# flair2005/image-analogies-python

Hardware: AMD Instinct MI355X
Metric: B' pixels synthesized/sec, exact NN, 1024² A/A'/B, 1/2/4/8 GPUs; % MFMA peak (higher is better)
Workload: dtype f16x3

## Files before the change

image-analogies-python_amd/_native.py:

```python
import ctypes
import math
import os
import threading

import numpy as np

_HERE = os.path.dirname(os.path.abspath(__file__))
LIB_PATH = os.environ.get('IA_LIBIA') or os.path.join(_HERE, 'libia.so')

IA_MEM_HOST, IA_MEM_DEVICE = 0, 1
IA_MATCH_F32, IA_MATCH_F16X3 = 0, 1
_ERRNAMES = {-1: 'IA_EINVAL', -2: 'IA_EHIP', -3: 'IA_ENOMEM', -4: 'IA_ENODEV', -5: 'IA_ECOMM'}


class IAError(RuntimeError):
    pass


class LevelArgs(ctypes.Structure):
    _fields_ = [('ch', ctypes.c_int), ('n_ap', ctypes.c_int), ('a_h', ctypes.c_int), ('a_w', ctypes.c_int),
                ('b_h', ctypes.c_int), ('b_w', ctypes.c_int),
                ('A', ctypes.c_void_p), ('Ac', ctypes.c_void_p), ('Ap', ctypes.c_void_p), ('Apc', ctypes.c_void_p),
                ('B', ctypes.c_void_p), ('Bc', ctypes.c_void_p), ('Bpc', ctypes.c_void_p), ('Bp', ctypes.c_void_p),
                ('weights', ctypes.c_void_p), ('kappa_factor', ctypes.c_double),
# ... 70 lines not shown
                                      ctypes.c_void_p]),
    'ia_index_destroy': (None, [ctypes.c_void_p]),
    'ia_coherence_batch': (ctypes.c_int, [ctypes.c_void_p, ctypes.c_void_p, ctypes.c_int64, ctypes.c_void_p,
                                          ctypes.c_void_p, ctypes.c_void_p, ctypes.c_int64, ctypes.c_int, ctypes.c_int,
                                          ctypes.c_int, ctypes.c_int, ctypes.c_void_p, ctypes.c_void_p,
                                          ctypes.c_void_p]),
    'ia_gaussian_pyramid': (ctypes.c_int, [ctypes.c_void_p, ctypes.c_void_p, ctypes.c_int, ctypes.c_int, ctypes.c_int,
                                           ctypes.c_int, ctypes.c_void_p, ctypes.c_void_p, ctypes.c_int]),
    'ia_color_matrix': (ctypes.c_int, [ctypes.c_void_p, ctypes.c_void_p, ctypes.c_int64, ctypes.c_void_p,
                                       ctypes.c_void_p, ctypes.c_int]),
    'ia_k3_microbench': (ctypes.c_int, [ctypes.c_void_p, ctypes.c_int64, ctypes.c_int, ctypes.c_int,
                                        ctypes.POINTER(ctypes.c_double)]),
    'ia_merge_winners': (ctypes.c_int, [ctypes.c_void_p, ctypes.c_void_p, ctypes.c_int, ctypes.c_int64,
                                        ctypes.c_void_p, ctypes.c_void_p]),
    'ia_chain_budget': (ctypes.c_int, [ctypes.c_int, ctypes.c_int, ctypes.c_int, ctypes.c_int]),
    'ia_wavefront_shape': (ctypes.c_int, [ctypes.c_int, ctypes.c_int, ctypes.POINTER(ctypes.c_int64),
                                          ctypes.POINTER(ctypes.c_int64)]),
    'ia_wavefront_step': (ctypes.c_int, [ctypes.c_int, ctypes.c_int, ctypes.c_int64, ctypes.POINTER(ctypes.c_int),
                                         ctypes.POINTER(ctypes.c_int)]),
    'ia_shard_tiles': (ctypes.c_int, [ctypes.c_int64, ctypes.c_int, ctypes.c_int, ctypes.POINTER(ctypes.c_int64),
                                      ctypes.POINTER(ctypes.c_int64)]),
    'ia_shard_tiles_pruned': (ctypes.c_int, [ctypes.c_int64, ctypes.c_int, ctypes.c_int,
                                             ctypes.POINTER(ctypes.c_int64), ctypes.POINTER(ctypes.c_int64)]),
    'ia_shard_morton_tile': (ctypes.c_int64, [ctypes.c_int64, ctypes.c_int64, ctypes.c_int]),
}

_lib = None
_lock = threading.Lock()


# ... 287 lines not shown
TILE_MUL = 2654435761


def shard_rows(n_rows, world, rank):
    t0, t1 = shard_tiles(n_rows, world, rank)
    nt = (n_rows + 31) // 32
    perm = np.arange(t0, t1, dtype=np.int64) * (TILE_MUL % nt) % nt
    rows = (np.arange(32)[:, None] * nt + perm[None, :]).ravel()
    return np.sort(rows[rows < n_rows])


def chain_budget(n_cu, vgprs, api_blocks_per_cu, wg_threads=64):
    return lib().ia_chain_budget(n_cu, vgprs, api_blocks_per_cu, wg_threads)


def wavefront_shape(h, w):
    s, m = ctypes.c_int64(), ctypes.c_int64()
    check(lib().ia_wavefront_shape(h, w, ctypes.byref(s), ctypes.byref(m)), 'ia_wavefront_shape')
    return s.value, m.value
```

image-analogies-python_amd/csrc/ia_capi.cpp:

```cpp
#include <hip/hip_runtime.h>
#include <rccl/rccl.h>

#include <algorithm>
#include <atomic>
#include <chrono>
#include <mutex>
#include <thread>
#include <cmath>
#include <cstdio>
#include <cstdlib>
#include <cstring>
#include <string>
#include <vector>

#include "../../include/ia.h"
#include "ia_internal.h"
#include "ia_launch.h"

#if IA_PROBE & 16
void ia_k3p_probe_dump();
#endif

namespace {

// ... 89 lines not shown
  int prune = 1;
  int row_source = 0;
  int shard_emulate = 1;
  int shard_unpruned = 0;
  int prune_group = 1;
  int matcher = IA_MATCH_F16X3;
  int k3p_variant = 24;
  int k3_variant = 1;
  int k3p_blocks = 1;
  int fuse_gather = 1;
  int fuse_unpruned = 0;
  HandSlot *hand = nullptr;
  int hand_rows = 0;
  int prefetch_next = 1;
  int early_gather = 1;
  int nn_bound = 1;
  int fuse_sort = 0;
  int chain_budget = 0;
  int scan_wgs = IA_NWG_H;
  unsigned long long *kslot = nullptr;
  int kslot_n = 0;
  unsigned hseq = 0;
  int time_dist = 0;
  int stamps = 0;
  int rec_wt = 1;
  DevBuf stamp_k3, stamp_mg, stamp_dur;
  std::vector<hipEvent_t> evs, evg, evm;
  hipEvent_t lv0 = nullptr, lv1 = nullptr, lv2 = nullptr;
  hipEvent_t kb[4] = {nullptr, nullptr, nullptr, nullptr};
  int rank = 0, world = 1;
// ... 273 lines not shown
  if (!std::strcmp(name, "fuse_gather")) {
    if (value != 0 && value != 1) return fail(IA_EINVAL, "ia_set_option: fuse_gather must be 0 or 1");
    c->fuse_gather = value;
    return IA_OK;
  }
  if (!std::strcmp(name, "nn_bound")) {
    if (value != 0 && value != 1) return fail(IA_EINVAL, "ia_set_option: nn_bound must be 0 or 1");
    c->nn_bound = value;
    return IA_OK;
  }
  if (!std::strcmp(name, "early_gather")) {
    if (value != 0 && value != 1) return fail(IA_EINVAL, "ia_set_option: early_gather must be 0 or 1");
    c->early_gather = value;
    return IA_OK;
  }
  if (!std::strcmp(name, "prefetch_next")) {
    if (value != 0 && value != 1) return fail(IA_EINVAL, "ia_set_option: prefetch_next must be 0 or 1");
    c->prefetch_next = value;
    return IA_OK;
  }
  if (!std::strcmp(name, "fuse_sort")) {
    if (value < 0 || value > 2) return fail(IA_EINVAL, "ia_set_option: fuse_sort must be 0, 1 or 2");
    c->fuse_sort = value;
    return IA_OK;
  }
  if (!std::strcmp(name, "fuse_unpruned")) {
    if (value != 0 && value != 1) return fail(IA_EINVAL, "ia_set_option: fuse_unpruned must be 0 or 1");
    c->fuse_unpruned = value;
    return IA_OK;
  }
// ... 156 lines not shown
  return IA_OK;
}

int ia_pipeline_generation(ia_ctx *c) { return c ? c->p_gen.load() : -1; }

int ia_chain_budget(int n_cu, int vgprs, int api_blocks_per_cu, int wg_threads) {
  if (n_cu <= 0 || vgprs <= 0 || api_blocks_per_cu <= 0 || wg_threads <= 0) return 0;
  const int alloc = (vgprs + 7) / 8 * 8;
  const int per_simd = alloc > 512 ? 0 : std::min(8, 512 / alloc);
  const int wpb = (wg_threads + IA_WAVE - 1) / IA_WAVE;
  int per_cu = std::min(4 * per_simd, api_blocks_per_cu * wpb);
  if (per_simd > 3) per_cu = std::min(per_cu, (api_blocks_per_cu - 1) * wpb);
  if (per_cu <= 0) return 0;
  const int slots = per_cu * n_cu;
  return 2 * slots - (2 * slots) / 16;
}
int ia_wavefront_shape(int h, int w, int64_t *steps, int64_t *max_queries) {
  if (h < 1 || w < 1) return fail(IA_EINVAL, "ia_wavefront_shape: empty level");
  if (steps) *steps = (int64_t)w + 3 * (int64_t)(h - 1);
  if (max_queries) *max_queries = std::min<int64_t>(h, (w + 2) / 3);
  return IA_OK;
}

int ia_wavefront_step(int h, int w, int64_t t, int *r0, int *M) {
  if (h < 1 || w < 1 || t < 0 || t >= (int64_t)w + 3 * (int64_t)(h - 1)) return fail(IA_EINVAL, "ia_wavefront_step: bad step");
  const int64_t r_lo = std::max<int64_t>(0, (t - w + 1 + 2) / 3);
  const int64_t r_hi = std::min<int64_t>(h - 1, t / 3);
  *r0 = (int)r_lo;
  *M = (int)(r_hi - r_lo + 1);
  return IA_OK;
// ... 558 lines not shown

struct LevelRun {
  ia_ctx *c;
  const LevelPlan &P;
  const LevelGeo &g;
  const LevelInputs &in;
  StampSlots &stamps;
  PipelineLink &link;
  ScanTally tally;
  double ufac;
  MergeArgs ma;
  std::vector<MergeArgs> mas;
  std::vector<int64_t> shard_rows;
  bool chain = false;
  ChainReservation &chain_res;
  bool fsort = false;
  int64_t gathered = -1;
  bool gsort = false;
  int64_t n_gm = 0;
  double gq_bytes = 0., gather_bytes_timed = 0.;

  LevelRun(ia_ctx *ctx, const LevelPlan &plan, const LevelInputs &inputs, StampSlots &s, PipelineLink &l, ChainReservation &r,
           double uf)
      : c(ctx), P(plan), g(plan.g), in(inputs), stamps(s), link(l), tally{ctx, plan.stride}, ufac(uf), chain_res(r) {}

  void init_merge_args() {
    const bool prune = P.prune, use_h = P.use_h;
    ma.db64 = c->db64.as<double>();
    ma.rec = c->rec.as<float4>();
    ma.recT = c->recT.as<float>();
// ... 32 lines not shown
      }
      for (int t = x.t0; t < x.t1 && !prune; t++) {
        const int64_t tr = ia_tile_perm(t, g.n_tiles);
        shard_rows[i] += std::min<int64_t>(IA_TILE, (g.NA - tr + g.n_tiles - 1) / g.n_tiles);
      }
    }
    gq_bytes = 55.0 * g.ch * 8 + (prune ? 12.0 * ia_db64_stride(g.ch) * 8 : 0.) + g.D * 8.0 +
               (use_h ? 16.0 * g.KS * 4 : P.DP * 4.0) + 8.0 + (prune ? 48.0 : 0.);
  }

  int init_chain() {
    static_assert(IA_NWG_H <= 4 * IA_WAVE, "k_merge_gather reads 4 records per lane");
    const int J = P.J;
    chain = c->fuse_gather && P.use_h && g.ch == 1 && g.bw >= 3 && (P.prune || c->fuse_unpruned) &&
            ((!P.multi && !P.xo && mas[0].nwg <= 4 * IA_WAVE) || (P.xo && P.prune));
    if (chain && !chain_res.take((int)(P.Mpad_max + J) + (P.xo ? 1 : 0), c->chain_budget)) chain = false;
    if (chain) {
      int rc;
      if ((rc = grow_uncached(c, (void **)&c->hand, &c->hand_rows, g.bh * J, sizeof(HandSlot))) ||
          (rc = grow_uncached(c, (void **)&c->kslot, &c->kslot_n, P.Mpad_max, 8)) || (rc = c->xerr.ensure(4)))
        return rc;
      HIP_TRY(hipMemsetAsync(c->xerr.p, 0, 4, c->st));
    }
    fsort = chain && P.prune && !P.xo && (c->fuse_sort == 1 || (c->fuse_sort == 2 && P.Mtmax >= IA_FUSE_SORT_MINQ)) &&
            g_chain_waves.load() <= c->chain_budget / 2;
    const int64_t n_timed = P.stride ? (P.T + P.stride - 1) / P.stride : 0;
    for (auto *v : {&c->evs, &c->evg, &c->evm})
      if ((int64_t)v->size() < 2 * n_timed) {
        size_t old = v->size();
        v->resize(2 * n_timed);
        for (size_t i = old; i < v->size(); i++) hipEventCreate(&(*v)[i]);
      }
    return IA_OK;
  }

  QBufs qhalf(int64_t t) const {
    const size_t h = chain && (t & 1) ? 1 : 0;
    return QBufs{c->q64.as<double>() + h * P.Mpad_max * g.D, c->qn2.as<double>() + h * P.Mpad_max,
                 P.prune ? c->qinfo.as<float4>() + h * 3 * P.Mpad_max : nullptr};
  }
// ... 10 lines not shown
    nx.sn = sn;
    const QBufs q = qhalf(sn.t);
    nx.q64 = q.q64 + q0n * g.D;
    nx.qn2 = q.qn2 + q0n;
    nx.qinfo = q.qinfo ? q.qinfo + 3 * q0n : nullptr;
    nx.qf = (char *)c->qf.p + q0n * P.db_row_bytes;
    nx.mu = c->mu.as<double>();
    nx.basis = c->pr_basis.as<double>();
    nx.ufac = ufac;
    nx.hand = c->hand + (size_t)jl * g.bh;
    nx.seq = ++c->hseq;
    nx.err = c->xerr.as<unsigned>();
    nx.timeout_ticks = IA_WAIT_TICKS;
    nx.prefetch = c->prefetch_next;
    nx.early = c->early_gather;
    return nx;
  }

  int step(int64_t t) {
    StepDesc sd;
    sd.t = (int)t;
    sd.J = P.J;
    ia_wavefront_step(g.bh, g.bw, t, &sd.r0, &sd.M);
    if (sd.M <= 0) return IA_OK;
    const int Mt = P.J * sd.M;
    sd.Mpad = (int)tile_pad(Mt);
    const bool timed_gm = P.stride && t % P.stride == 0;
    if (timed_gm) {
      hipEventRecord(c->evg[2 * n_gm], c->st);
      gather_bytes_timed += gq_bytes * Mt;
// ... 857 lines not shown
```

image-analogies-python_amd/csrc/ia_gather.h:

```cpp
#pragma once
#include "ia_dev.h"

template <int KS>
__device__ __forceinline__ void put_qh(_Float16 *qf, int m, int f, double v) {
  const int qt = m / IA_TILE, j = m % IA_TILE, s = f >> 4, h = (f >> 3) & 1, e = f & 7;
  _Float16 hi, lo;
  split_h(v, hi, lo);
  const int64_t base = (((int64_t)qt * 2 * KS + 2 * s) * IA_WAVE + h * IA_TILE + j) * 8 + e;
  qf[base] = hi;
  qf[base + IA_WAVE * 8] = lo;
}

struct QHand {
  int r0 = -1, c0 = -1, r1 = -1, c1 = -1;
  double v0 = 0., v1 = 0.;
  int s0r = 0, s0c = 0, i0 = 0, s1r = 0, s1c = 0, i1 = 0;
  int n0 = -1, n1 = -1;
};
template <bool FUSE>
__device__ __forceinline__ double feat_q1(const Imgs &B, int f, int r, int c, const QHand &h) {
  if constexpr (FUSE) {
    if (f >= 43) {
      const int k = f - 43, y = ia_reflect(r + k / 5 - 2, B.h), x = ia_reflect(c + k % 5 - 2, B.w);
      if (y == h.r0 && x == h.c0) return h.v0;
// ... 401 lines not shown
    nx.qn2[mn] = ss;
    nx.qinfo[3 * mn] = make_float4(round_down_f(p[0] - IA_PRUNE_MABS), round_down_f(p[1] - IA_PRUNE_MABS),
                                   round_down_f(p[2] - IA_PRUNE_MABS), round_down_f(p[3] - IA_PRUNE_MABS));
    nx.qinfo[3 * mn + 1] = make_float4(round_up_f(p[0] + IA_PRUNE_MABS), round_up_f(p[1] + IA_PRUNE_MABS),
                                       round_up_f(p[2] + IA_PRUNE_MABS), round_up_f(p[3] + IA_PRUNE_MABS));
    nx.qinfo[3 * mn + 2] = make_float4(up, __uint_as_float(key), z, w);
  }
  IA_GST2(5);
#if IA_PROBE & 8
  if (gprobe && lane == 0)
    printf("ESTAMP bw=%d t=%d M=%d pre=%llu part=%llu handoff=%llu late=%llu rec=%llu\n", g.bw, sn.t, sn.M, gst[1] - gst[0],
           gst[2] - gst[1], gst[3] - gst[2], gst[4] - gst[3], gst[5] - gst[4]);
#endif
#undef IA_GST2
}
```

image-analogies-python_amd/csrc/ia_internal.h:

```cpp
#pragma once
#include <hip/hip_runtime.h>
#include <stdint.h>

#define IA_WAVE 64
#define IA_TILE 32
#define IA_WG 256
#define IA_MAX_D 168
#define IA_WG_TARGET 512
#define IA_PAD_NORM 1.0e30f
#define IA_WGH 512
#define IA_NWG_H 256
#define IA_NORM_SCALE 256.0
#define IA_F16_MAXABS 64.0

template <int KS>
struct TileFmt {
  static constexpr bool CMP = KS == 4;
  static constexpr int STRIDE = CMP ? (2 * KS - 2) * IA_WAVE + 2 * IA_TILE : 2 * KS * IA_WAVE;
  __host__ __device__ static constexpr int off(int p, int L) {
    return (CMP && p >= 2 * KS - 2) ? (2 * KS - 2) * IA_WAVE + (p - (2 * KS - 2)) * IA_TILE + (L & 31) : p * IA_WAVE + L;
  }
};
#define IA_MATCH_F32 0
#define IA_MATCH_F16X3 1
// ... 212 lines not shown
  const double *mu, *basis;
  double *q64, *qn2;
  void *qf;
  float4 *qinfo;
  double ufac;
  HandSlot *hand;
  unsigned seq;
  unsigned *err;
  long long timeout_ticks;
  XOPub xp;
  const unsigned *wait_seq;
  int wait_n;
  unsigned long long *kslot;
  int prefetch;
  int early;
  int *sorder;
  float4 *sinfo;
  void *sfrag;
};

__host__ __device__ inline int ia_reflect(int i, int n) {
  int j = i < 0 ? -i - 1 : i;
  j = j >= n ? 2 * n - 1 - j : j;
  if ((unsigned)j < (unsigned)n) return j;
  const int m = 2 * n;
  i %= m;
  if (i < 0) i += m;
  return i >= n ? m - 1 - i : i;
}

// ... 12 lines not shown
```

image-analogies-python_amd/csrc/ia_kernels.hip:

```cpp
#include "ia_certify.h"
#include "ia_gather.h"
#include "ia_launch.h"

#if IA_PROBE & 8
#define IA_STAMP(k) do { __builtin_amdgcn_sched_barrier(0); stamp[k] = __builtin_amdgcn_s_memtime(); \
                         __builtin_amdgcn_sched_barrier(0); } while (0)
#else
#define IA_STAMP(k) do { } while (0)
#endif

struct MergeOut {
  double v;
  int pr, pc, img;
  int nn;
};

struct NoPre {
  __device__ __forceinline__ void operator()() const {}
};
template <int CH, int RPL, class Pre = NoPre>
__device__ __forceinline__ void merge_fused(const LevelGeo &g, const StepDesc &sd, const Imgs &A, const MergeArgs &a,
                                            int m, const JobPtrs &jp, const QPix &px,
                                            double *qs, double *ws, int *cand_row, float *cand_v,
                                            MergeOut *out = nullptr, Pre pre = Pre{}) {
#if IA_PROBE & 8
  unsigned long long stamp[8] = {0, 0, 0, 0, 0, 0, 0, 0};
#endif
  IA_STAMP(0);
  constexpr int NCOH = 15, NRR = IA_WAVE - NCOH;
  const int lane = threadIdx.x & 63;
  const int r = px.r, c = px.c, qi = px.qi;
  int32_t *__restrict__ s = jp.s, *__restrict__ im = jp.im;
  double *__restrict__ Bp = jp.Bp;
// ... 88 lines not shown
    const int pos = placed + lane_prefix(bal);
    if (cmask != 0 && pos < NRR) {
      float v;
      cand_row[pos] = lowest_cand<RPL>(cmask, i1, i2, v1, v2, v);
      cand_v[pos] = v;
      cmask &= cmask - 1;
    }
    placed += __popcll(bal);
    bal = __ballot(cmask != 0);
  }
  const int n_cand = min(placed, NRR);
  __builtin_amdgcn_wave_barrier();
  int my_row = lane < NCOH ? crow : (lane - NCOH < n_cand ? cand_row[lane - NCOH] : -1);
  const float my_v = lane >= NCOH && my_row >= 0 ? cand_v[lane - NCOH] : FLT_MAX;
  IA_STAMP(2);
  pre();

  double unw = DBL_MAX, wsq = 0.;
  double av[CH];
#pragma unroll
  for (int k = 0; k < CH; k++) av[k] = 0.;
  if (my_row >= 0) {
    const unsigned img = (unsigned)my_row / hw;
    const double *src = A.p3 + img * A.img_stride_f + (int64_t)((unsigned)my_row - img * hw) * CH;
#pragma unroll
    for (int k = 0; k < CH; k++) av[k] = src[k];
    row_dists<CH>(a.db64, my_row, qs, ws, unw, wsq);
  }
  const bool viol = lane >= NCOH && my_row >= 0 && fabs(unw - qn2 - (double)my_v) > eps + 1e-13 * (unw + qn2);
  const bool any_viol = __ballot(viol) != 0;
#if IA_PROBE & 8
// ... 169 lines not shown
      o[1] = app_pc;
      o[2] = app_img;
      o[3] = has_coh ? r - 2 + kk / 5 : 0;
      o[4] = has_coh ? c - 2 + kk % 5 : 0;
      o[5] = has_coh ? 1 : 0;
      jp.dbg_dist[2 * qi] = dbg_app;
      jp.dbg_dist[2 * qi + 1] = dbg_coh;
    }
  }
  if (out) {
    out->v = val[0];
    out->pr = pr;
    out->pc = pc;
    out->img = img;
    out->nn = bi >= 0 && bi < a.NA ? bi : -1;
  }
#if IA_PROBE & 8
  if (lane == 0 && m == sd.M / 2 && (sd.t % 256) == 128) {
    __builtin_amdgcn_s_waitcnt(0);
    const unsigned long long t7 = __builtin_amdgcn_s_memtime();
    printf("STAMP bw=%d t=%d M=%d slot=%d nfb=%d d1=%llu d2=%llu d3=%llu d4=%llu d5=%llu d6=%llu d7=%llu\n", g.bw, sd.t,
           sd.M, placed, (int)nfb, stamp[1] - stamp[0], stamp[2] - stamp[1], stamp[3] - stamp[2], stamp[4] - stamp[3],
           stamp[5] - stamp[4], stamp[6] - stamp[5], t7 - stamp[6]);
  }
#endif
}

template <int CH, bool FUSED, class JS, int RPL = IA_WG_TARGET / IA_WAVE>
__global__ void __launch_bounds__(IA_PQ_WG) k_merge_level(LevelGeo g, StepDesc sd, Imgs A, MergeArgs ma, Winner *__restrict__ win,
                                                        JS jobs) {
// ... 8 lines not shown
    const int wv = threadIdx.x >> 6;
    const unsigned long long t0 = ma.stamp ? ia_clock() : 0ull;
    merge_fused<CH, RPL>(g, sd, A, ma, m, jp, px, qsh[wv], wsh[wv], crsh[wv], cvsh[wv]);
    if (ma.stamp && (threadIdx.x & 63) == 0) ia_stamp_wg(ma.stamp, t0);
  } else {
    const double *q = ma.q64 + (int64_t)m * Geo<CH>::D;
    unsigned stat = 0;
    const Winner wn = certified_winner<RPL>(ma, m, [&](int64_t row) { return exact_dist_level<CH>(ma.db64, row, q); }, &stat);
    if ((threadIdx.x & 63) == 0) {
      win[m] = wn;
      if (jp.pstat) jp.pstat[px.qi] = stat;
    }
  }
}

template <int RPL, bool PR, bool XO, class JS>
__device__ __forceinline__ void merge_gather_body(const LevelGeo &g, const StepDesc &sd, const Imgs &A, const MergeArgs &ma,
                                                  const JS &jobs, Imgs B, const NextStep &nx) {
  constexpr int KS = 4;
  const int w = __builtin_amdgcn_readfirstlane(blockIdx.x * IA_PQ_WPB + (threadIdx.x >> 6));
  const int lane = threadIdx.x & 63, wv = threadIdx.x >> 6;
  const int J = JS::single ? 1 : sd.J, JM = J * sd.M;
  __shared__ double qsh[IA_PQ_WPB][Geo<1>::DS], wsh[IA_PQ_WPB][Geo<1>::DS];
  __shared__ int crsh[IA_PQ_WPB][IA_WAVE];
  __shared__ float cvsh[IA_PQ_WPB][IA_WAVE];
  __shared__ __attribute__((aligned(16))) _Float16 xh[IA_PQ_WPB][2][16 * KS];
  if (XO && w >= JM + J + (nx.sn.Mpad - J * nx.sn.M)) {
    if (__hip_atomic_load(nx.err, __ATOMIC_RELAXED, __HIP_MEMORY_SCOPE_AGENT)) return;
    const long long t0 = (long long)__builtin_amdgcn_s_memrealtime();
    for (int i = lane; i < nx.wait_n; i += IA_WAVE)
      while (__hip_atomic_load(nx.wait_seq + i, __ATOMIC_RELAXED, __HIP_MEMORY_SCOPE_SYSTEM) != nx.xp.seq) {
        if ((long long)__builtin_amdgcn_s_memrealtime() - t0 > nx.timeout_ticks) {
          atomicOr(nx.err, 4u);
          break;
        }
        __builtin_amdgcn_s_sleep(2);
      }
    return;
  }
  QHand h;
  int mn = -1;
  int job = 0;
  QPre pf;
  const bool early = PR && !XO && !nx.kslot && nx.prefetch && nx.early;
  QConst qk;
  if (early) qk = qconst_load(nx, lane);
#if IA_PROBE & 8
  unsigned long long gs[5] = {__builtin_amdgcn_s_memtime(), 0, 0, 0, 0}, gst[5] = {0, 0, 0, 0, 0};
  const bool gprobe = w == sd.M / 2 && (sd.t % 256) == 128 && JM == sd.M;
#endif
  if (w < JM) {
    const QPix px = ia_qpix(sd, g.bw, w);
    job = px.job;
    const JobPtrs jp = jobs.get(job);
    MergeOut o;
    if (px.c + 1 < g.bw) mn = job * nx.sn.M + (px.r - nx.sn.r0);
    const Imgs Bj = JS::single ? B : job_imgs(B, jp);
    auto pre = [&]() {
      if (PR && nx.prefetch && mn >= 0) pf = qpre_load(g, nx.sn, Bj, jp, mn, lane);
    };
    merge_fused<1, RPL>(g, sd, A, ma, w, jp, px, qsh[wv], wsh[wv], crsh[wv], cvsh[wv], &o, pre);
    if (px.r + 1 < g.bh && px.c >= 2) {
      HandSlot *hs = nx.hand + (int64_t)job * g.bh + px.r;
      if (lane == 0) {
        hs->v = o.v;
        hs->sr = o.pr;
        hs->sc = o.pc;
        hs->im = o.img;
        hs->nn = o.nn;
      }
      ia_stores_done();
      if (lane == 0) __hip_atomic_store(&hs->seq, nx.seq, __ATOMIC_RELAXED, __HIP_MEMORY_SCOPE_SYSTEM);
    }
// ... 73 lines not shown
                             );
    if (XO && nx.xp.W) xo_publish<KS>(nx.xp, mn, lane, xh[wv][0], xh[wv][1], o0, o1, o2);
    if (!XO && nx.kslot) sorted_publish<KS>(nx, mn, lane, xh[wv][0], xh[wv][1], o0, o1, o2);
  } else {
    gather_h_query_fused<KS>(g, nx.sn, B, mn, lane, nx.mu, nx.q64, nx.qn2, qf, h);
  }
#if IA_PROBE & 8
  __builtin_amdgcn_s_waitcnt(0);
  gs[3] = __builtin_amdgcn_s_memtime();
  if (gprobe && lane == 0)
    printf("GSTAMP bw=%d t=%d M=%d merge=%llu handoff_wait=%llu gather=%llu [feat+frag=%llu sums=%llu urow=%llu rec=%llu]\n",
           g.bw, sd.t, sd.M, gs[1] - gs[0], gs[2] - gs[1], gs[3] - gs[2], gst[1] - gst[0], gst[2] - gst[1], gst[3] - gst[2],
           gst[4] - gst[3]);
#endif
}
template <int RPL, bool PR, bool XO, class JS>
__global__ void __launch_bounds__(IA_PQ_WG) k_merge_gather(LevelGeo g, StepDesc sd, Imgs A, MergeArgs ma, JS jobs,
                                                         Imgs B, NextStep nx) {
  const unsigned long long t0 = ma.stamp ? ia_clock() : 0ull;
  merge_gather_body<RPL, PR, XO, JS>(g, sd, A, ma, jobs, B, nx);
  if (ma.stamp && (threadIdx.x & 63) == 0) ia_stamp_wg(ma.stamp, t0);
}

void ia_launch_merge(const LevelGeo &g, const StepDesc &sd, const Imgs &A, const MergeArgs &ma, Winner *win,
                     const JobSet &jobs, bool fused, hipStream_t st) {
  const dim3 grid(cdiv(sd.J * sd.M, IA_PQ_WPB));
  const bool r4 = fused && ma.nwg <= 4 * IA_WAVE;
  with_ch(g.ch, [&](auto c) {
    with_jobs(jobs, [&](auto js) {
      constexpr int CH = decltype(c)::CH;
      using JS = decltype(js);
      if (r4) hipLaunchKernelGGL((k_merge_level<CH, true, JS, 4>), grid, dim3(IA_PQ_WG), 0, st, g, sd, A, ma, win, js);
      else if (fused) hipLaunchKernelGGL((k_merge_level<CH, true, JS>), grid, dim3(IA_PQ_WG), 0, st, g, sd, A, ma, win, js);
      else hipLaunchKernelGGL((k_merge_level<CH, false, JS>), grid, dim3(IA_PQ_WG), 0, st, g, sd, A, ma, win, js);
    });
  });
}

struct MergeGatherInst {
  bool single, pruned, xo;
  const void *fn;
};
static const MergeGatherInst k_merge_gather_insts[] = {
    {true, true, true, (const void *)k_merge_gather<4, true, true, JobArg1>},
    {true, true, false, (const void *)k_merge_gather<4, true, false, JobArg1>},
    {true, false, false, (const void *)k_merge_gather<4, false, false, JobArg1>},
    {false, true, false, (const void *)k_merge_gather<4, true, false, JobArgN>},
    {false, false, false, (const void *)k_merge_gather<4, false, false, JobArgN>},
};

void ia_launch_merge_gather(const LevelGeo &g, const StepDesc &sd, const Imgs &A, const MergeArgs &ma, const JobSet &jobs,
                            const Imgs &B, const NextStep &nx, bool pruned, hipStream_t st) {
  const int nw = sd.J * sd.M + sd.J + (nx.sn.Mpad - sd.J * nx.sn.M) + (nx.wait_n > 0 ? 1 : 0);
  const dim3 grid(cdiv(nw, IA_PQ_WPB));
  const bool single = jobs.J == 1;
  const bool xo = single && pruned && (nx.xp.W > 0 || nx.wait_n > 0);
  for (const MergeGatherInst &k : k_merge_gather_insts) {
    if (k.single != single || k.pruned != pruned || k.xo != xo) continue;
    JobArg1 j1{jobs.j0};
    JobArgN jn{jobs.rest};
    Imgs Bj = single ? job0_imgs(B, jobs) : B;
    void *args[] = {(void *)&g,  (void *)&sd, (void *)&A, (void *)&ma, single ? (void *)&j1 : (void *)&jn,
                    (void *)&Bj, (void *)&nx};
    (void)hipLaunchKernel(k.fn, grid, dim3(IA_PQ_WG), args, 0, st);
    return;
  }
}
void ia_merge_gather_occupancy(int *vgprs, int *blocks_per_cu, int *wg_threads) {
  int vmax = 0, bmin = 1 << 30;
  for (const MergeGatherInst &k : k_merge_gather_insts) {
    hipFuncAttributes fa;
    int nb = 0;
    if (hipFuncGetAttributes(&fa, k.fn) != hipSuccess ||
        hipOccupancyMaxActiveBlocksPerMultiprocessor(&nb, k.fn, IA_PQ_WG, 0) != hipSuccess) {
      bmin = 0;
      continue;
    }
    vmax = std::max(vmax, (int)fa.numRegs);
    bmin = std::min(bmin, nb);
  }
  *vgprs = vmax;
  *blocks_per_cu = bmin;
  *wg_threads = IA_PQ_WG;
}
```

include/ia.h:

```cpp
#ifndef IA_H_
#define IA_H_

#include <stdint.h>

#ifdef __cplusplus
extern "C" {
#endif

#define IA_OK 0
#define IA_EINVAL -1
#define IA_EHIP -2
#define IA_ENOMEM -3
#define IA_ENODEV -4
#define IA_ECOMM -5

#define IA_MEM_HOST 0
#define IA_MEM_DEVICE 1

typedef struct ia_ctx ia_ctx;
typedef struct ia_index ia_index;

typedef struct {
  int64_t pixels;
  int64_t steps;
// ... 90 lines not shown
void ia_index_destroy(ia_index *index);
int ia_coherence_batch(ia_index *index, const double *q, int64_t nq, const int32_t *px,
                       const int32_t *s, const int32_t *im, int64_t n_s, int a_h, int a_w,
                       int bp_w, int pad, int32_t *p_out, int32_t *img_out, int32_t *rstar_out);

int ia_gaussian_pyramid(ia_ctx *ctx, const double *img, int h, int w, int ch, int n_reduce,
                        const double *weights7, double *out, int mem);
int ia_color_matrix(ia_ctx *ctx, const double *in, int64_t npx, const double *M9, double *out,
                    int mem);

int ia_k3_microbench(ia_ctx *ctx, int64_t n_rows, int M, int reps, double *us_per_launch);

int ia_merge_winners(const double *dist, const int64_t *row, int world, int64_t nq,
                     double *dist_out, int64_t *row_out);
int ia_chain_budget(int n_cu, int vgprs, int api_blocks_per_cu, int wg_threads);
int ia_wavefront_shape(int h, int w, int64_t *steps, int64_t *max_queries);
int ia_wavefront_step(int h, int w, int64_t t, int *r0, int *M);
int ia_shard_tiles(int64_t n_rows, int world, int rank, int64_t *tile0, int64_t *tile1);
int ia_shard_tiles_pruned(int64_t n_rows, int world, int rank, int64_t *tile0, int64_t *tile1);
int64_t ia_shard_morton_tile(int64_t storage_tile, int64_t n_tiles, int world);

#ifdef __cplusplus
}
#endif
#endif
```

Measured before the change: 5.771 million.

## Add two-wave merge/gather kernel form overlapping next-query gather with merge

```diff
diff --git a/image-analogies-python_amd/_native.py b/image-analogies-python_amd/_native.py
--- a/image-analogies-python_amd/_native.py
+++ b/image-analogies-python_amd/_native.py
@@ -108,6 +108,7 @@
     'ia_merge_winners': (ctypes.c_int, [ctypes.c_void_p, ctypes.c_void_p, ctypes.c_int, ctypes.c_int64,
                                         ctypes.c_void_p, ctypes.c_void_p]),
     'ia_chain_budget': (ctypes.c_int, [ctypes.c_int, ctypes.c_int, ctypes.c_int, ctypes.c_int]),
+    'ia_chain_choice': (ctypes.c_int, [ctypes.c_int, ctypes.c_int, ctypes.c_int, ctypes.c_int]),
     'ia_wavefront_shape': (ctypes.c_int, [ctypes.c_int, ctypes.c_int, ctypes.POINTER(ctypes.c_int64),
                                           ctypes.POINTER(ctypes.c_int64)]),
     'ia_wavefront_step': (ctypes.c_int, [ctypes.c_int, ctypes.c_int, ctypes.c_int64, ctypes.POINTER(ctypes.c_int),
@@ -425,6 +426,10 @@
     return lib().ia_chain_budget(n_cu, vgprs, api_blocks_per_cu, wg_threads)
 
 
+def chain_choice(level_waves, in_flight, budget, two_wave=1):
+    return lib().ia_chain_choice(level_waves, in_flight, budget, two_wave)
+
+
 def wavefront_shape(h, w):
     s, m = ctypes.c_int64(), ctypes.c_int64()
     check(lib().ia_wavefront_shape(h, w, ctypes.byref(s), ctypes.byref(m)), 'ia_wavefront_shape')
diff --git a/image-analogies-python_amd/csrc/ia_capi.cpp b/image-analogies-python_amd/csrc/ia_capi.cpp
--- a/image-analogies-python_amd/csrc/ia_capi.cpp
+++ b/image-analogies-python_amd/csrc/ia_capi.cpp
@@ -127,6 +127,7 @@
   int hand_rows = 0;
   int prefetch_next = 1;
   int early_gather = 1;
+  int gather_wave = 1;
   int nn_bound = 1;
   int fuse_sort = 0;
   int chain_budget = 0;
@@ -430,6 +431,11 @@
     c->early_gather = value;
     return IA_OK;
   }
+  if (!std::strcmp(name, "gather_wave")) {
+    if (value != 0 && value != 1) return fail(IA_EINVAL, "ia_set_option: gather_wave must be 0 or 1");
+    c->gather_wave = value;
+    return IA_OK;
+  }
   if (!std::strcmp(name, "prefetch_next")) {
     if (value != 0 && value != 1) return fail(IA_EINVAL, "ia_set_option: prefetch_next must be 0 or 1");
     c->prefetch_next = value;
@@ -616,6 +622,12 @@
   if (per_cu <= 0) return 0;
   const int slots = per_cu * n_cu;
   return 2 * slots - (2 * slots) / 16;
+}
+int ia_chain_choice(int level_waves, int in_flight, int budget, int two_wave) {
+  if (level_waves <= 0 || in_flight < 0 || budget <= 0) return 0;
+  const int64_t left = (int64_t)budget - in_flight;
+  if (two_wave && 2 * (int64_t)level_waves <= left) return 2;
+  return level_waves <= left ? 1 : 0;
 }
 int ia_wavefront_shape(int h, int w, int64_t *steps, int64_t *max_queries) {
   if (h < 1 || w < 1) return fail(IA_EINVAL, "ia_wavefront_shape: empty level");
@@ -1204,6 +1216,7 @@
   std::vector<int64_t> shard_rows;
   bool chain = false;
   ChainReservation &chain_res;
+  bool gwave = false;
   bool fsort = false;
   int64_t gathered = -1;
   bool gsort = false;
@@ -1266,7 +1279,15 @@
     const int J = P.J;
     chain = c->fuse_gather && P.use_h && g.ch == 1 && g.bw >= 3 && (P.prune || c->fuse_unpruned) &&
             ((!P.multi && !P.xo && mas[0].nwg <= 4 * IA_WAVE) || (P.xo && P.prune));
-    if (chain && !chain_res.take((int)(P.Mpad_max + J) + (P.xo ? 1 : 0), c->chain_budget)) chain = false;
+    const bool want_sort = P.prune && !P.xo && (c->fuse_sort == 1 || (c->fuse_sort == 2 && P.Mtmax >= IA_FUSE_SORT_MINQ));
+    const bool two = c->gather_wave && c->early_gather && c->prefetch_next && P.prune && !P.multi && !P.xo && J == 1 && !want_sort;
+    if (chain) {
+      const int lw = (int)(P.Mpad_max + J) + (P.xo ? 1 : 0);
+      int form = ia_chain_choice(lw, g_chain_waves.load(), c->chain_budget, two);
+      while (form && !chain_res.take(form * lw, c->chain_budget)) form--;
+      chain = form > 0;
+      gwave = form == 2;
+    }
     if (chain) {
       int rc;
       if ((rc = grow_uncached(c, (void **)&c->hand, &c->hand_rows, g.bh * J, sizeof(HandSlot))) ||
@@ -1274,8 +1295,7 @@
         return rc;
       HIP_TRY(hipMemsetAsync(c->xerr.p, 0, 4, c->st));
     }
-    fsort = chain && P.prune && !P.xo && (c->fuse_sort == 1 || (c->fuse_sort == 2 && P.Mtmax >= IA_FUSE_SORT_MINQ)) &&
-            g_chain_waves.load() <= c->chain_budget / 2;
+    fsort = chain && want_sort && g_chain_waves.load() <= c->chain_budget / 2;
     const int64_t n_timed = P.stride ? (P.T + P.stride - 1) / P.stride : 0;
     for (auto *v : {&c->evs, &c->evg, &c->evm})
       if ((int64_t)v->size() < 2 * n_timed) {
@@ -1316,6 +1336,7 @@
     nx.timeout_ticks = IA_WAIT_TICKS;
     nx.prefetch = c->prefetch_next;
     nx.early = c->early_gather;
+    nx.gwave = gwave;
     return nx;
   }
 
diff --git a/image-analogies-python_amd/csrc/ia_gather.h b/image-analogies-python_amd/csrc/ia_gather.h
--- a/image-analogies-python_amd/csrc/ia_gather.h
+++ b/image-analogies-python_amd/csrc/ia_gather.h
@@ -439,3 +439,219 @@
 #endif
 #undef IA_GST2
 }
+
+struct GatherWave {
+  QConst qk;
+  bool late0 = false, late1 = false;
+  bool own = false;
+  unsigned long long lm0 = 0, lm1 = 0;
+  int crow = -1;
+  double qc = 0., ss = 0., p[IA_NPC] = {0., 0., 0., 0.};
+  double part = 0., al[12] = {0., 0., 0., 0., 0., 0., 0., 0., 0., 0., 0., 0.};
+  int row2 = -1;
+  double part2 = 0., al2[12] = {0., 0., 0., 0., 0., 0., 0., 0., 0., 0., 0., 0.};
+#if IA_PROBE & 8
+  unsigned long long t0 = 0, t1 = 0, t2 = 0;
+#endif
+};
+__device__ __forceinline__ void gather_wave_row(const double *__restrict__ db64, int crow, const double *qsh,
+                                                unsigned long long lm, double &part, double *al) {
+  constexpr int D = 55, DS = Geo<1>::DS;
+  double2 rowv[DS / 2];
+  const double2 *src = reinterpret_cast<const double2 *>(db64 + (int64_t)(crow >= 0 ? crow : 0) * DS);
+#pragma unroll
+  for (int i = 0; i < DS / 2; i++) rowv[i] = src[i];
+  const double *rv = reinterpret_cast<const double *>(rowv);
+  part = pw_sum<D>([&](int f) {
+    const double d = rv[f] - qsh[f];
+    return ((lm >> f) & 1ull) ? 0. : d * d;
+  });
+#pragma unroll
+  for (int k = 0; k < 12; k++) al[k] = rv[43 + k];
+}
+template <int KS>
+__device__ __forceinline__ GatherWave gather_wave_pre(const LevelGeo &g, const NextStep &nx, const Imgs &B, const JobPtrs &jp,
+                                                      int mn, int lane, const double *__restrict__ db64, double *qsh) {
+  constexpr int D = 55, KD = 16 * KS;
+  static_assert(KD <= IA_WAVE, "one feature per lane");
+  GatherWave w;
+#if IA_PROBE & 8
+  w.t0 = __builtin_amdgcn_s_memtime();
+#endif
+  w.qk = qconst_load(nx, lane);
+  const QPre pf = qpre_load(g, nx.sn, B, jp, mn, lane);
+  const QPix pn = ia_qpix(nx.sn, g.bw, mn);
+  const int r = pn.r, c = pn.c, qi = pn.qi;
+  const bool above = r >= 1 && c + 2 < g.bw;
+  const int ar = r - 1, ac = c + 2, orr = r, oc = c - 1;
+  if (lane >= 43 && lane < D) {
+    const int k = lane - 43, y = ia_reflect(r + k / 5 - 2, B.h), x = ia_reflect(c + k % 5 - 2, B.w);
+    w.late0 = y == orr && x == oc;
+    w.late1 = above && y == ar && x == ac;
+  }
+  w.lm0 = __ballot(w.late0);
+  w.lm1 = __ballot(w.late1);
+  const bool late = w.late0 || w.late1;
+  const bool nnl = jp.nn && lane >= 15 && lane < 30;
+  if (qi > 0 && (lane < 15 || nnl)) {
+    const int k = lane < 15 ? lane : lane - 15;
+    const int nr = r - 2 + k / 5, nc = c - 2 + k % 5;
+    if (nr >= 0 && nc >= 0 && nc < g.bw && nr * g.bw + nc < qi && !(above && nr == ar && nc == ac)) {
+      if (nr == orr && nc == oc) w.own = true;
+      else w.crow = ucand_row(g, r, c, nr, nc, nnl, pf.sr, pf.sc, pf.si, pf.nn);
+    }
+  }
+  if (lane < D) qsh[lane] = late ? 0. : pf.v;
+  if (lane < KD) {
+    if (lane < D) {
+      if (!late) {
+        nx.q64[(int64_t)mn * D + lane] = pf.v;
+        w.qc = pf.v - w.qk.mu;
+        w.ss = w.qc * w.qc;
+        put_qh<KS>((_Float16 *)nx.qf, mn, lane, -2.0 * w.qc);
+#pragma unroll
+        for (int i = 0; i < IA_NPC; i++) w.p[i] = w.qk.bas[i] * w.qc;
+      }
+    } else {
+      put_qh<KS>((_Float16 *)nx.qf, mn, lane, lane == D ? IA_NORM_SCALE : 0.);
+    }
+  }
+  w.ss = wave_sum_d_x(w.ss);
+#pragma unroll
+  for (int i = 0; i < IA_NPC; i++) w.p[i] = wave_sum_d_x(w.p[i]);
+  __builtin_amdgcn_wave_barrier();
+#if IA_PROBE & 8
+  __builtin_amdgcn_s_waitcnt(0);
+  w.t1 = __builtin_amdgcn_s_memtime();
+#endif
+  gather_wave_row(db64, w.crow, qsh, w.lm0 | w.lm1, w.part, w.al);
+#if IA_PROBE & 8
+  __builtin_amdgcn_s_waitcnt(0);
+  w.t2 = __builtin_amdgcn_s_memtime();
+#endif
+  return w;
+}
+__device__ __forceinline__ void gather_wave_next(const LevelGeo &g, const NextStep &nx, const int *prow, int *prow_on,
+                                                 int lane, const double *__restrict__ db64, const double *qsh,
+                                                 GatherWave &w) {
+  const long long t0 = (long long)__builtin_amdgcn_s_memrealtime();
+  bool ok = true;
+  while (__hip_atomic_load(prow_on, __ATOMIC_ACQUIRE, __HIP_MEMORY_SCOPE_WORKGROUP) != 1) {
+    if ((long long)__builtin_amdgcn_s_memrealtime() - t0 > nx.timeout_ticks) {
+      atomicOr(nx.err, 16u);
+      ok = false;
+      break;
+    }
+    __builtin_amdgcn_s_sleep(1);
+  }
+  if (ok) {
+    const int mr = prow[lane];
+    if (mr >= 0 && mr < g.NA && (unsigned)mr % (unsigned)g.aw + 1 < (unsigned)g.aw) w.row2 = mr + 1;
+  }
+  gather_wave_row(db64, w.row2, qsh, w.lm0 | w.lm1, w.part2, w.al2);
+#if IA_PROBE & 8
+  __builtin_amdgcn_s_waitcnt(0);
+  w.t2 = __builtin_amdgcn_s_memtime();
+#endif
+}
+__device__ __forceinline__ void gather_wave_late(GatherWave &w, unsigned long long lm, double v) {
+#pragma unroll
+  for (int k = 0; k < 12; k++) {
+    if ((lm >> (43 + k)) & 1ull) {
+      const double qcl = readlane_d(w.qc, 43 + k);
+      w.ss += qcl * qcl;
+#pragma unroll
+      for (int i = 0; i < IA_NPC; i++) w.p[i] += readlane_d(w.qk.bas[i], 43 + k) * qcl;
+      const double d = w.al[k] - v;
+      w.part += d * d;
+    }
+  }
+}
+template <int KS>
+__device__ __forceinline__ void gather_wave_post(const LevelGeo &g, const NextStep &nx, const JobPtrs &jp, int job, int mn,
+                                                 int lane, const double *__restrict__ db64, const double *qsh, const QHand &h,
+                                                 int src_lane, int app_lane, GatherWave &w) {
+  constexpr int D = 55;
+#if IA_PROBE & 8
+  unsigned long long gst[5] = {__builtin_amdgcn_s_memtime(), 0, 0, 0, 0};
+  const bool gprobe = mn == nx.sn.M / 2 && (nx.sn.t % 256) == 129;
+#define IA_GST3(k) do { if (gprobe) { __builtin_amdgcn_s_waitcnt(0); __builtin_amdgcn_sched_barrier(0); \
+                        gst[k] = __builtin_amdgcn_s_memtime(); __builtin_amdgcn_sched_barrier(0); } } while (0)
+#else
+#define IA_GST3(k) do { } while (0)
+#endif
+  const QPix pn = ia_qpix(nx.sn, g.bw, mn);
+  const int r = pn.r, c = pn.c;
+  const bool above = r >= 1 && c + 2 < g.bw;
+  const int from = lane < 15 ? src_lane : app_lane;
+  const int fl = from >= 0 ? from : lane;
+  const int row2 = __shfl(w.row2, fl, 64);
+  const double part2 = __shfl(w.part2, fl, 64);
+  double al2[12];
+#pragma unroll
+  for (int k = 0; k < 12; k++) al2[k] = __shfl(w.al2[k], fl, 64);
+  if (w.own) {
+    w.crow = ucand_row(g, r, c, h.r0, h.c0, lane >= 15, h.s0r, h.s0c, h.i0, h.n0);
+    if (from >= 0 && row2 == w.crow) {
+      w.part = part2;
+#pragma unroll
+      for (int k = 0; k < 12; k++) w.al[k] = al2[k];
+    } else {
+      gather_wave_row(db64, w.crow, qsh, w.lm0 | w.lm1, w.part, w.al);
+    }
+  }
+  if (w.late0) {
+    nx.q64[(int64_t)mn * D + lane] = h.v0;
+    w.qc = h.v0 - w.qk.mu;
+    put_qh<KS>((_Float16 *)nx.qf, mn, lane, -2.0 * w.qc);
+  }
+  gather_wave_late(w, w.lm0, h.v0);
+  IA_GST3(1);
+  if (above) {
+    const HandSlot *hs = nx.hand + (int64_t)job * g.bh + (r - 1);
+    const long long t0 = (long long)__builtin_amdgcn_s_memrealtime();
+    while (__hip_atomic_load(&hs->seq, __ATOMIC_RELAXED, __HIP_MEMORY_SCOPE_SYSTEM) != nx.seq) {
+      if ((long long)__builtin_amdgcn_s_memrealtime() - t0 > nx.timeout_ticks) {
+        atomicOr(nx.err, 16u);
+        break;
+      }
+      __builtin_amdgcn_s_sleep(1);
+    }
+    const double v1 = hs->v;
+    IA_GST3(2);
+    if (w.late1) {
+      nx.q64[(int64_t)mn * D + lane] = v1;
+      w.qc = v1 - w.qk.mu;
+      put_qh<KS>((_Float16 *)nx.qf, mn, lane, -2.0 * w.qc);
+    }
+    gather_wave_late(w, w.lm1, v1);
+  } else {
+    IA_GST3(2);
+  }
+  double u = w.crow >= 0 ? w.part : DBL_MAX;
+  u = wave_min_d_x(u);
+  IA_GST3(3);
+  const double ss = w.ss, qn = sqrt(ss);
+  const double(&p)[IA_NPC] = w.p;
+  const bool fin = u < DBL_MAX;
+  const unsigned key = fin ? prune_key(p, w.qk.sc) : IA_PRUNE_KEY_INF;
+  const float up = fin ? round_up_f(u * nx.ufac) : INFINITY;
+  const float z = fin ? round_up_f((double)up - ss + 0x1p-22 * (ss + (double)up) + 0x1p-24 * (16.0 * qn + 300.0)) : INFINITY;
+  const float wd = round_up_f(0x1p-8 * qn * (1.0 + 0x1p-40));
+  if (lane == 0) {
+    nx.qn2[mn] = ss;
+    nx.qinfo[3 * mn] = make_float4(round_down_f(p[0] - IA_PRUNE_MABS), round_down_f(p[1] - IA_PRUNE_MABS),
+                                   round_down_f(p[2] - IA_PRUNE_MABS), round_down_f(p[3] - IA_PRUNE_MABS));
+    nx.qinfo[3 * mn + 1] = make_float4(round_up_f(p[0] + IA_PRUNE_MABS), round_up_f(p[1] + IA_PRUNE_MABS),
+                                       round_up_f(p[2] + IA_PRUNE_MABS), round_up_f(p[3] + IA_PRUNE_MABS));
+    nx.qinfo[3 * mn + 2] = make_float4(up, __uint_as_float(key), z, wd);
+  }
+  IA_GST3(4);
+#if IA_PROBE & 8
+  if (gprobe && lane == 0)
+    printf("WSTAMP bw=%d t=%d M=%d pre=%llu part=%llu wait_merge=%llu own=%llu handoff=%llu late=%llu rec=%llu\n", g.bw,
+           nx.sn.t, nx.sn.M, w.t1 - w.t0, w.t2 - w.t1, gst[0] - w.t2, gst[1] - gst[0], gst[2] - gst[1], gst[3] - gst[2],
+           gst[4] - gst[3]);
+#endif
+#undef IA_GST3
+}
diff --git a/image-analogies-python_amd/csrc/ia_internal.h b/image-analogies-python_amd/csrc/ia_internal.h
--- a/image-analogies-python_amd/csrc/ia_internal.h
+++ b/image-analogies-python_amd/csrc/ia_internal.h
@@ -250,6 +250,7 @@
   unsigned long long *kslot;
   int prefetch;
   int early;
+  int gwave;
   int *sorder;
   float4 *sinfo;
   void *sfrag;
diff --git a/image-analogies-python_amd/csrc/ia_kernels.hip b/image-analogies-python_amd/csrc/ia_kernels.hip
--- a/image-analogies-python_amd/csrc/ia_kernels.hip
+++ b/image-analogies-python_amd/csrc/ia_kernels.hip
@@ -13,10 +13,11 @@
   double v;
   int pr, pc, img;
   int nn;
+  int src_lane, app_lane;
 };
 
 struct NoPre {
-  __device__ __forceinline__ void operator()() const {}
+  __device__ __forceinline__ void operator()(int) const {}
 };
 template <int CH, int RPL, class Pre = NoPre>
 __device__ __forceinline__ void merge_fused(const LevelGeo &g, const StepDesc &sd, const Imgs &A, const MergeArgs &a,
@@ -135,7 +136,7 @@
   int my_row = lane < NCOH ? crow : (lane - NCOH < n_cand ? cand_row[lane - NCOH] : -1);
   const float my_v = lane >= NCOH && my_row >= 0 ? cand_v[lane - NCOH] : FLT_MAX;
   IA_STAMP(2);
-  pre();
+  pre(my_row);
 
   double unw = DBL_MAX, wsq = 0.;
   double av[CH];
@@ -335,6 +336,8 @@
     out->pc = pc;
     out->img = img;
     out->nn = bi >= 0 && bi < a.NA ? bi : -1;
+    out->src_lane = src_lane;
+    out->app_lane = recompute_app ? -1 : app_lane;
   }
 #if IA_PROBE & 8
   if (lane == 0 && m == sd.M / 2 && (sd.t % 256) == 128) {
@@ -373,17 +376,83 @@
   }
 }
 
-template <int RPL, bool PR, bool XO, class JS>
+template <int RPL>
+__device__ __forceinline__ void merge_gather_pair(const LevelGeo &g, const StepDesc &sd, const Imgs &A, const MergeArgs &ma,
+                                                  const JobPtrs &jp, const Imgs &B, const NextStep &nx, int w, int role,
+                                                  int lane, double *qsh, double *wsh, int *crsh, float *cvsh) {
+  constexpr int KS = 4;
+  __shared__ double gq[Geo<1>::DS];
+  __shared__ MergeOut mo;
+  const QPix px = ia_qpix(sd, g.bw, w);
+  const int mn = px.c + 1 < g.bw ? px.r - nx.sn.r0 : -1;
+  const bool on = mn >= 0 && mn < nx.sn.M;
+  __shared__ int prow[IA_WAVE];
+  __shared__ int prow_on;
+  if (role == 0 && lane == 0) __hip_atomic_store(&prow_on, 0, __ATOMIC_RELAXED, __HIP_MEMORY_SCOPE_WORKGROUP);
+  __syncthreads();
+  GatherWave gw;
+  MergeOut o;
+  if (role == 0) {
+    auto post = [&](int my_row) {
+      prow[lane] = my_row;
+      __builtin_amdgcn_wave_barrier();
+      if (lane == 0) __hip_atomic_store(&prow_on, 1, __ATOMIC_RELEASE, __HIP_MEMORY_SCOPE_WORKGROUP);
+    };
+    merge_fused<1, RPL>(g, sd, A, ma, w, jp, px, qsh, wsh, crsh, cvsh, &o, post);
+    if (lane == 0) mo = o;
+  } else if (on) {
+    gw = gather_wave_pre<KS>(g, nx, B, jp, mn, lane, ma.db64, gq);
+    gather_wave_next(g, nx, prow, &prow_on, lane, ma.db64, gq, gw);
+  }
+  __syncthreads();
+  if (role == 0) {
+    if (px.r + 1 < g.bh && px.c >= 2) {
+      HandSlot *hs = nx.hand + px.r;
+      if (lane == 0) {
+        hs->v = o.v;
+        hs->sr = o.pr;
+        hs->sc = o.pc;
+        hs->im = o.img;
+        hs->nn = o.nn;
+      }
+      ia_stores_done();
+      if (lane == 0) __hip_atomic_store(&hs->seq, nx.seq, __ATOMIC_RELAXED, __HIP_MEMORY_SCOPE_SYSTEM);
+    }
+    return;
+  }
+  if (!on) return;
+  QHand h;
+  h.r0 = px.r;
+  h.c0 = px.c;
+  h.v0 = mo.v;
+  h.s0r = __builtin_amdgcn_readfirstlane(mo.pr);
+  h.s0c = __builtin_amdgcn_readfirstlane(mo.pc);
+  h.i0 = __builtin_amdgcn_readfirstlane(mo.img);
+  h.n0 = __builtin_amdgcn_readfirstlane(mo.nn);
+  gather_wave_post<KS>(g, nx, jp, 0, mn, lane, ma.db64, gq, h, __builtin_amdgcn_readfirstlane(mo.src_lane),
+                       __builtin_amdgcn_readfirstlane(mo.app_lane), gw);
+}
+
+template <int RPL, bool PR, bool XO, class JS, bool GW = false>
 __device__ __forceinline__ void merge_gather_body(const LevelGeo &g, const StepDesc &sd, const Imgs &A, const MergeArgs &ma,
                                                   const JS &jobs, Imgs B, const NextStep &nx) {
   constexpr int KS = 4;
-  const int w = __builtin_amdgcn_readfirstlane(blockIdx.x * IA_PQ_WPB + (threadIdx.x >> 6));
-  const int lane = threadIdx.x & 63, wv = threadIdx.x >> 6;
+  static_assert(!GW || (PR && !XO && JS::single && IA_PQ_WPB == 1), "two-wave form: the one-job pruned early path");
+  const int w = __builtin_amdgcn_readfirstlane(GW ? blockIdx.x : blockIdx.x * IA_PQ_WPB + (threadIdx.x >> 6));
+  const int lane = threadIdx.x & 63, wv = GW ? 0 : threadIdx.x >> 6;
   const int J = JS::single ? 1 : sd.J, JM = J * sd.M;
   __shared__ double qsh[IA_PQ_WPB][Geo<1>::DS], wsh[IA_PQ_WPB][Geo<1>::DS];
   __shared__ int crsh[IA_PQ_WPB][IA_WAVE];
   __shared__ float cvsh[IA_PQ_WPB][IA_WAVE];
   __shared__ __attribute__((aligned(16))) _Float16 xh[IA_PQ_WPB][2][16 * KS];
+  if constexpr (GW) {
+    const int role = __builtin_amdgcn_readfirstlane(threadIdx.x >> 6);
+    if (w < JM) {
+      merge_gather_pair<RPL>(g, sd, A, ma, jobs.get(0), B, nx, w, role, lane, qsh[0], wsh[0], crsh[0], cvsh[0]);
+      return;
+    }
+    if (role) return;
+  }
   if (XO && w >= JM + J + (nx.sn.Mpad - J * nx.sn.M)) {
     if (__hip_atomic_load(nx.err, __ATOMIC_RELAXED, __HIP_MEMORY_SCOPE_AGENT)) return;
     const long long t0 = (long long)__builtin_amdgcn_s_memrealtime();
@@ -408,14 +477,14 @@
   unsigned long long gs[5] = {__builtin_amdgcn_s_memtime(), 0, 0, 0, 0}, gst[5] = {0, 0, 0, 0, 0};
   const bool gprobe = w == sd.M / 2 && (sd.t % 256) == 128 && JM == sd.M;
 #endif
-  if (w < JM) {
+  if (!GW && w < JM) {
     const QPix px = ia_qpix(sd, g.bw, w);
     job = px.job;
     const JobPtrs jp = jobs.get(job);
     MergeOut o;
     if (px.c + 1 < g.bw) mn = job * nx.sn.M + (px.r - nx.sn.r0);
     const Imgs Bj = JS::single ? B : job_imgs(B, jp);
-    auto pre = [&]() {
+    auto pre = [&](int) {
       if (PR && nx.prefetch && mn >= 0) pf = qpre_load(g, nx.sn, Bj, jp, mn, lane);
     };
     merge_fused<1, RPL>(g, sd, A, ma, w, jp, px, qsh[wv], wsh[wv], crsh[wv], cvsh[wv], &o, pre);
@@ -519,11 +588,11 @@
            gst[4] - gst[3]);
 #endif
 }
-template <int RPL, bool PR, bool XO, class JS>
-__global__ void __launch_bounds__(IA_PQ_WG) k_merge_gather(LevelGeo g, StepDesc sd, Imgs A, MergeArgs ma, JS jobs,
-                                                         Imgs B, NextStep nx) {
+template <int RPL, bool PR, bool XO, class JS, bool GW = false>
+__global__ void __launch_bounds__(GW ? 2 * IA_WAVE : IA_PQ_WG)
+k_merge_gather(LevelGeo g, StepDesc sd, Imgs A, MergeArgs ma, JS jobs, Imgs B, NextStep nx) {
   const unsigned long long t0 = ma.stamp ? ia_clock() : 0ull;
-  merge_gather_body<RPL, PR, XO, JS>(g, sd, A, ma, jobs, B, nx);
+  merge_gather_body<RPL, PR, XO, JS, GW>(g, sd, A, ma, jobs, B, nx);
   if (ma.stamp && (threadIdx.x & 63) == 0) ia_stamp_wg(ma.stamp, t0);
 }
 
@@ -543,48 +612,55 @@
 }
 
 struct MergeGatherInst {
-  bool single, pruned, xo;
+  bool single, pruned, xo, gw;
   const void *fn;
+  int threads() const { return gw ? 2 * IA_WAVE : IA_PQ_WG; }
 };
 static const MergeGatherInst k_merge_gather_insts[] = {
-    {true, true, true, (const void *)k_merge_gather<4, true, true, JobArg1>},
-    {true, true, false, (const void *)k_merge_gather<4, true, false, JobArg1>},
-    {true, false, false, (const void *)k_merge_gather<4, false, false, JobArg1>},
-    {false, true, false, (const void *)k_merge_gather<4, true, false, JobArgN>},
-    {false, false, false, (const void *)k_merge_gather<4, false, false, JobArgN>},
+    {true, true, true, false, (const void *)k_merge_gather<4, true, true, JobArg1>},
+    {true, true, false, false, (const void *)k_merge_gather<4, true, false, JobArg1>},
+    {true, true, false, true, (const void *)k_merge_gather<4, true, false, JobArg1, true>},
+    {true, false, false, false, (const void *)k_merge_gather<4, false, false, JobArg1>},
+    {false, true, false, false, (const void *)k_merge_gather<4, true, false, JobArgN>},
+    {false, false, false, false, (const void *)k_merge_gather<4, false, false, JobArgN>},
 };
 
 void ia_launch_merge_gather(const LevelGeo &g, const StepDesc &sd, const Imgs &A, const MergeArgs &ma, const JobSet &jobs,
                             const Imgs &B, const NextStep &nx, bool pruned, hipStream_t st) {
   const int nw = sd.J * sd.M + sd.J + (nx.sn.Mpad - sd.J * nx.sn.M) + (nx.wait_n > 0 ? 1 : 0);
-  const dim3 grid(cdiv(nw, IA_PQ_WPB));
   const bool single = jobs.J == 1;
   const bool xo = single && pruned && (nx.xp.W > 0 || nx.wait_n > 0);
+  const bool gw = nx.gwave && single && pruned && !xo && !nx.kslot && nx.prefetch && nx.early;
   for (const MergeGatherInst &k : k_merge_gather_insts) {
-    if (k.single != single || k.pruned != pruned || k.xo != xo) continue;
+    if (k.single != single || k.pruned != pruned || k.xo != xo || k.gw != gw) continue;
+    const dim3 grid(gw ? nw : cdiv(nw, IA_PQ_WPB));
     JobArg1 j1{jobs.j0};
     JobArgN jn{jobs.rest};
     Imgs Bj = single ? job0_imgs(B, jobs) : B;
     void *args[] = {(void *)&g,  (void *)&sd, (void *)&A, (void *)&ma, single ? (void *)&j1 : (void *)&jn,
                     (void *)&Bj, (void *)&nx};
-    (void)hipLaunchKernel(k.fn, grid, dim3(IA_PQ_WG), args, 0, st);
+    (void)hipLaunchKernel(k.fn, grid, dim3(k.threads()), args, 0, st);
     return;
   }
 }
 void ia_merge_gather_occupancy(int *vgprs, int *blocks_per_cu, int *wg_threads) {
-  int vmax = 0, bmin = 1 << 30;
+  int vmax = 0, wmin = 1 << 30;
+  *blocks_per_cu = 0;
+  *wg_threads = IA_PQ_WG;
   for (const MergeGatherInst &k : k_merge_gather_insts) {
     hipFuncAttributes fa;
     int nb = 0;
     if (hipFuncGetAttributes(&fa, k.fn) != hipSuccess ||
-        hipOccupancyMaxActiveBlocksPerMultiprocessor(&nb, k.fn, IA_PQ_WG, 0) != hipSuccess) {
-      bmin = 0;
-      continue;
-    }
-    vmax = std::max(vmax, (int)fa.numRegs);
-    bmin = std::min(bmin, nb);
+        hipOccupancyMaxActiveBlocksPerMultiprocessor(&nb, k.fn, k.threads(), 0) != hipSuccess)
+      nb = 0;
+    else
+      vmax = std::max(vmax, (int)fa.numRegs);
+    const int waves = nb * (k.threads() / IA_WAVE);
+    if (waves < wmin) {
+      wmin = waves;
+      *blocks_per_cu = nb;
+      *wg_threads = k.threads();
+    }
   }
   *vgprs = vmax;
-  *blocks_per_cu = bmin;
-  *wg_threads = IA_PQ_WG;
-}
+}
diff --git a/include/ia.h b/include/ia.h
--- a/include/ia.h
+++ b/include/ia.h
@@ -128,6 +128,7 @@
 int ia_merge_winners(const double *dist, const int64_t *row, int world, int64_t nq,
                      double *dist_out, int64_t *row_out);
 int ia_chain_budget(int n_cu, int vgprs, int api_blocks_per_cu, int wg_threads);
+int ia_chain_choice(int level_waves, int in_flight, int budget, int two_wave);
 int ia_wavefront_shape(int h, int w, int64_t *steps, int64_t *max_queries);
 int ia_wavefront_step(int h, int w, int64_t t, int *r0, int *M);
 int ia_shard_tiles(int64_t n_rows, int world, int rank, int64_t *tile0, int64_t *tile1);
```

After: 5.860 million (median of 6 runs). 1.02x the previous value.
